# md-k-sarker/azure-hc-intel-tf

Measured on AMD Instinct MI355X. Metric: images/sec (whole node) ResNet-50 bs=64/worker at 1/2/4/8 MI355X, higher is better.
Workload: dtype fp32; 1 GPU; model=resnet50, global_batch=64, per_gpu_batch=64, image_size=224, parallelism=dp1, optimizer=momentum(0.9)+wd4e-5, fp32 master, graph=True, backward_segments=stage, kernels=hip

## Files before the change

### azure_hc_intel_tf_amd/ops/autotune.py

```python
from __future__ import annotations

import json
import math
import os
from typing import Dict, List, Tuple

import torch

from . import _ext
from . import functional as Fn

_DIR = os.path.join(os.path.dirname(os.path.dirname(os.path.abspath(__file__))), "tuned")


def _table_path(v):
    if not v or os.path.isabs(v) or os.path.exists(v):
        return v
    alt = os.path.join(os.path.dirname(os.path.dirname(os.path.dirname(os.path.abspath(__file__)))), v)
    return alt if os.path.exists(alt) else v


DEFAULT_CACHE = _table_path(os.environ.get("HCB_TUNED_TABLE")) or os.path.join(_DIR, "mi355x.json")
CACHE_VERSION = 6


def _entry_valid(key, val) -> bool:
    tiles = {"fwd": Fn._CONV_TILES, "dgb": Fn._CONV_TILES, "wgrad": Fn._WGRAD_TILES, "fwd3": Fn._P3_TILES,
             "wgrad3": Fn._WP3_TILES}.get(key[0])
    cfg, splits = (val[0], val[1]) if isinstance(val, (tuple, list)) else (val, 1)
    return tiles is not None and int(cfg) in tiles and int(splits) >= 1


def _key_str(k) -> str:
    return "|".join(str(v) for v in k)


def _key_parse(s: str):
    parts = s.split("|")
    return (parts[0],) + tuple(int(p) for p in parts[1:])


def load_cache(path: str = DEFAULT_CACHE) -> int:
    if not os.path.exists(path):
        return 0
    with open(path) as f:
        d = json.load(f)
    if d.get("version") != CACHE_VERSION:
        return 0
    table = {}
    for k, v in d.get("entries", {}).items():
        key, val = _key_parse(k), tuple(v) if isinstance(v, list) else v
        if _entry_valid(key, val):
# ... 117 lines not shown


def layer_problems_p3(layer, batch: int, dev) -> List[Tuple]:
    spec = layer.spec
    H, W, Cin = layer.in_shape
    P, Q, Cout = layer.out_shape
    N = batch
    M = N * P * Q
    taps = spec.kh * spec.kw
    geo = Fn.dgrad_problem(spec, N, H, W, P, Q)
    phases = Fn.dgrad_phases(spec, H, W) if layer.need_dx and Fn.uses_dgrad_phases(spec, H, W) else []
    buf = {}

    def ops():
        if not buf:
            buf["x"] = _planes((N, H, W, Cin), dev)
            buf["dz"] = _planes((N, P, Q, Cout), dev)
            buf["y"] = torch.empty((N, P, Q, Cout), dtype=torch.float32, device=dev)
            buf["acc"] = torch.zeros(8 * 2 * Cout, dtype=torch.float32, device=dev)
            buf["dx"] = torch.zeros((N, H, W, Cin), dtype=torch.float32, device=dev)
            buf["dw"] = torch.zeros((Cout, spec.K), dtype=torch.float32, device=dev)
        return buf

    out = [(Fn.fwd3_key(M, Cout, spec.K, taps), [list(c) for c in Fn.p3_candidates(M, Cout, spec.K)],
            lambda plan: Fn.conv_forward(ops()["x"], spec, layer.pack.pack, None, ops()["y"], stats=ops()["acc"],
                                         cfg=plan, stats_R=8))]
    if layer.need_dx:
        if not phases:
            out.append((Fn.fwd3_key(geo[0], Cin, geo[1], taps), [list(c) for c in Fn.p3_candidates(geo[0], Cin, geo[1])],
                        lambda plan: Fn.conv_dgrad(ops()["dz"], spec, layer.pack.tr, None, ops()["dx"], False,
                                                   cfg=plan)))
        for ph in phases:
            pm, pk, pt = Fn.dgrad_phase_problem(spec, N, ph)
            out.append((Fn.fwd3_key(pm, Cin, pk, pt), [list(c) for c in Fn.p3_candidates(pm, Cin, pk)],
                        lambda plan, ph=ph: Fn.dgrad_phase(ops()["dz"], spec, layer.pack.tr, ops()["dx"], True, ph,
                                                           cfg=plan)))
    out.append((Fn.wgrad3_key(Cout, spec.K, M, taps), [list(c) for c in Fn.wgrad_p3_candidates(Cout, spec.K, M)],
                lambda plan: Fn.conv_wgrad(ops()["dz"], ops()["x"], spec, ops()["dw"], cfg=tuple(plan))))
    return out


def _best(cands, run):
    best = None
    for plan in cands:
        t = _time(lambda: run(plan))
        if best is None or t < best[0]:
            best = (t, plan)
    return best


def model_problems(model, batch: int):
    from ..nn.layers import ConvBN
# ... 63 lines not shown
```

### azure_hc_intel_tf_amd/ops/functional.py

```python
from __future__ import annotations

import math
import os
from dataclasses import dataclass
from typing import NamedTuple

import torch
import torch.nn.functional as F

from . import _ext


def ld(t) -> int:
    if t.dim() == 4:
        assert t.stride(3) == 1, "activation channels must be contiguous"
        return t.stride(2)
    assert t.dim() == 2 and t.stride(1) == 1
    return t.stride(0)


def _round_up(x: int, m: int) -> int:
    return (x + m - 1) // m * m


# ... 428 lines not shown


def dgrad_problem(spec, N, H, W, P, Q):
    return dgrad_geom(spec, N, H, W, P, Q, 0, 0)[1][:2]


def set_tuned(table: dict) -> None:
    _tuned.update(table)


_P3_TILES = {0: (128, 64), 1: (64, 128), 2: (128, 64), 3: (64, 128), 4: (64, 64), 5: (128, 64), 6: (64, 128),
             7: (128, 128), 8: (128, 128), 9: (128, 128), 10: (256, 128), 11: (128, 256), 12: (64, 128),
             13: (128, 64), 14: (128, 64), 15: (64, 128), 16: (64, 64), 17: (64, 64),
             18: (64, 128), 19: (128, 64), 20: (64, 64), 21: (64, 64), 22: (128, 128),
             23: (64, 128), 24: (128, 64), 25: (64, 64), 26: (64, 64), 27: (128, 128), 28: (128, 128),
             31: (64, 256), 32: (128, 256), 33: (64, 64), 34: (128, 64),
             35: (128, 64), 36: (128, 128)}
_P3_OCC = {14: 2, 15: 2, 16: 2, 17: 3, 18: 2, 19: 2, 20: 2, 21: 3, 23: 2, 24: 2, 25: 2, 26: 3}
_P3_PERSIST = {18: 15, 19: 14, 20: 16, 21: 17, 22: 7, 23: 15, 24: 14, 25: 16, 26: 17, 27: 7, 28: 8,
               31: 15, 32: 15, 33: 16, 34: 14, 35: 14, 36: 7}
_P3_BRES = {31: 3, 32: 2, 33: 3, 34: 2, 35: 2, 36: 2}


def p3_bres_fits(cfg: int, N: int, K: int) -> bool:
    bm, bn = _P3_TILES[cfg]
    kpad = -(-K // 64) * 64
    return _P3_BRES[cfg] * 3 * bm * 64 + kpad * 3 * bn * 2 + 4 * N <= 160 * 1024
_P3_STREAMK = {23: 18, 24: 19, 25: 20, 26: 21, 27: 22, 28: 8}
_WP3_TILES = {0: (128, 64), 1: (64, 128), 2: (64, 64), 3: (128, 64), 4: (64, 128), 5: (64, 64),
              6: (128, 128), 7: (128, 128), 8: (256, 128), 9: (128, 256), 10: (128, 128), 11: (128, 64),
              12: (128, 64), 13: (64, 128), 14: (64, 64), 15: (64, 64),
              16: (128, 64), 17: (64, 128), 18: (64, 64)}
_WP3_OCC = {12: 2, 13: 2, 14: 2, 15: 3, 16: 2, 17: 2, 18: 3}


def fwd3_key(M: int, N: int, K: int, taps: int = 1):
    return ("fwd3", M, N, K, taps)


def wgrad3_key(Nout: int, K: int, M: int, taps: int = 1):
    return ("wgrad3", Nout, K, M, taps)


def p3_candidates(M: int, N: int, K: int):
    out = []
    ksteps = math.ceil(K / 64)
# ... 310 lines not shown

    def __init__(self, mean, invstd):
        self.mean = mean
        self.invstd = invstd


def conv_bn_inference(x, spec: ConvSpec, wpack, w_master, gamma, beta, running_mean, running_var, eps, out,
                      relu: bool, residual=None, cfg=None):
    N, H, W, _ = x.shape
    P, Q = spec.out_hw(H, W)
    M = N * P * Q
    p3 = is_planes(x) or (native(x) and x.dtype == torch.float32)
    if not p3 and not native(x):
        z = torch.empty((N, P, Q, spec.cout), dtype=out.dtype, device=x.device)
        conv_forward(x, spec, wpack, w_master, z)
        return bn_inference(z, gamma, beta, running_mean, running_var, eps, out, relu, residual=residual)
    if p3:
        x = to_planes(x)
        assert out.dtype == torch.float32, "fp32 conv needs an fp32 (or Planes) output"
        if residual is not None:
            residual = to_planes(residual) if is_planes(out) else from_planes(residual)
    cfg, splits = _plan(cfg, M, spec.cout, spec.K, x.device, spec.kh * spec.kw, **(_P3_PLAN if p3 else {}))
    if p3:
        cfg = _P3_PERSIST.get(cfg, cfg)
    elif cfg in PATCH_CFGS:
        cfg, splits = _PATCH_TWIN[cfg], 1
    if residual is not None:
        assert ld(residual) == ld(out) and residual.shape == out.shape and residual.dtype == out.dtype
    geom = fwd_geom(spec, N, H, W, ld(x), ld(out), residual is not None, not is_planes(out) and _f32o(out), relu)
    _launch(x, wpack, out, geom, cfg, splits, yres=residual, inf=(gamma, beta, running_mean, running_var, float(eps)))
    return out


def bn_inference(z, gamma, beta, running_mean, running_var, eps, out, relu: bool, residual=None):
    N, H, W, C = z.shape
    if native(z) and z.dtype == torch.float32:
        M = N * H * W
        acc = torch.stack([torch.zeros_like(running_var), running_var * float(M)]).unsqueeze(0).contiguous()
        scratch = torch.empty(2, C, dtype=torch.float32, device=z.device)
        if residual is not None:
            if is_planes(out) and not is_planes(residual):
                residual = to_planes(residual)
            elif not is_planes(out) and is_planes(residual):
                residual = from_planes(residual)
        _ext.ops().bn_apply_acc(z, ld(z), _pl(out), ld(out), _pl(residual), ld(residual) if residual is not None else 0,
                                M, C, acc, 1, eps, 1.0, gamma, beta, 1 if relu else 0, scratch[0], scratch[1],
                                None, None, running_mean)
# ... 390 lines not shown
```

### csrc/bindings.cpp

```cpp
#include <algorithm>
#include <vector>

#include <torch/library.h>
#include <ATen/core/Tensor.h>
#include <ATen/ops/empty.h>
#include <c10/hip/HIPStream.h>
#include <c10/util/Exception.h>

#include "kernels/kernels.h"

using at::Tensor;

#ifdef HCB_F16
constexpr at::ScalarType kAct = at::kHalf;
#define HCB_ACT_NAME "float16"
#else
constexpr at::ScalarType kAct = at::kBFloat16;
#define HCB_ACT_NAME "bfloat16"
#endif
#define HCB_TORCH_LIBRARY(ns, m) TORCH_LIBRARY(ns, m)
#define HCB_TORCH_LIBRARY_IMPL(ns, k, m) TORCH_LIBRARY_IMPL(ns, k, m)

namespace {

// ... 276 lines not shown
    TORCH_CHECK(t->dim() == 1 && t->numel() == p.Nout && t->is_contiguous() && t->device() == y.device(),
                "hcb.conv_inf: gamma / beta / moving mean / moving variance must be fp32 [cout] on the output's device");
  }
  p.bnb_gamma = gamma.data_ptr<float>();
  p.bnb_beta = beta.data_ptr<float>();
  p.bnb_mean = mean.data_ptr<float>();
  p.bnb_invstd = var.data_ptr<float>();
  p.inf = 1;
  p.inf_eps = (float)eps;
}

void conv_igemm_inf(const Tensor& x, const Tensor& w, const Tensor& y, const c10::optional<Tensor>& res,
                    at::IntArrayRef g, int64_t cfg, const Tensor& gamma, const Tensor& beta, const Tensor& mean,
                    const Tensor& var, double eps) {
  TORCH_CHECK(hcb::conv_cfg_has_inf((int)cfg), "hcb.conv_igemm_inf: cfg 0..16 (a patch cfg runs its LDS-DMA twin)");
  hcb::ConvParams p = igemm_params(x, w, y, res, c10::nullopt, c10::nullopt, g, cfg);
  TORCH_CHECK(x.scalar_type() != at::kFloat && !p.out_f32,
              "hcb.conv_igemm_inf: 16-bit operands and output (fp32 runs on the plane GEMMs: hcb.conv_p3_inf)");
  TORCH_CHECK(!p.beta || res->scalar_type() == y.scalar_type(), "hcb.conv_igemm_inf: res dtype differs from y");
  set_inf(p, y, gamma, beta, mean, var, eps);
  hcb::launch_conv_igemm(p, (int)cfg, cur_stream());
}

std::vector<int64_t> gemm_cfg_table(std::string family) {
  const hcb::GemmCfg* rows = nullptr;
  int n = 0;
  bool (*inf)(int) = [](int) { return false; };
  if (family == "conv") {
    rows = hcb::CONV_CFGS, n = hcb::N_CONV_CFG, inf = hcb::conv_cfg_has_inf;
  } else if (family == "wgrad") {
    rows = hcb::WGRAD_CFGS, n = hcb::N_WGRAD_CFG;
  } else if (family == "p3") {
    rows = hcb::P3_CFGS, n = hcb::N_P3_CFG, inf = hcb::p3_cfg_has_inf;
  } else if (family == "wgrad_p3") {
    rows = hcb::WP3_CFGS, n = hcb::N_WP3_CFG;
  } else {
    TORCH_CHECK(false, "hcb.gemm_cfg_table: family is conv, wgrad, p3 or wgrad_p3");
  }
  std::vector<int64_t> out;
  for (int i = 0; i < n; ++i) {
    const hcb::GemmCfg& r = rows[i];
    for (int v : {r.cfg, r.kind, r.wm, r.wn, r.tm, r.tn, r.kw, r.nst, r.occ, r.extra, r.fb, (int)inf(i)}) out.push_back(v);
  }
  return out;
}

int wgrad_params(hcb::WgradParams& p, const Tensor& dy, const Tensor& x, const Tensor& dw, at::IntArrayRef g,
                 int64_t splits, const char* op) {
  p = decode_geom(kWgradGeom, g, op);
  check_f32(dw, "dw");
  p.K = p.R * p.S * p.C;
  TORCH_CHECK(p.C % 8 == 0 && p.ldx % 8 == 0, "hcb.", op, ": C, ldx multiples of 8");
  TORCH_CHECK(p.ldy % 8 == 0 && p.ldy >= p.Nout, "hcb.", op, ": bad ldy");
  TORCH_CHECK(splits >= 1, "hcb.", op, ": splits >= 1");
  const int64_t xb = x_span_bytes(p.N, p.H, p.W, p.C, p.ldx, 2);
  const int64_t yb = out_span_bytes(p.M, p.ldy, p.Nout, 2);
  TORCH_CHECK(xb < (1ll << 31) && yb < (1ll << 31), "hcb.", op, ": operand exceeds 2 GiB");
  check_range(dw, (int64_t)p.Nout * p.K * 4, "dw");
  const int nkt = (p.M + 63) / 64;
  const int per = (nkt + (int)splits - 1) / (int)splits;
// ... 686 lines not shown
  const bool p3 = wp.dim() == 3 && wp.size(0) == 3 && wp.scalar_type() == at::kBFloat16;
  TORCH_CHECK((p3 || wp.scalar_type() == kAct) && wp.is_contiguous() && wp.numel() == (p3 ? 3 : 1) * w.size(0) * 256,
              "hcb.stem_wfold: wp bf16 [cout][256] or planes [3][cout][256]");
  hcb::launch_stem_wfold(w.data_ptr<float>(), (int)w.size(0), (int)w.size(3),
                         reinterpret_cast<uint16_t*>(wp.data_ptr()), cur_stream(), p3);
}

void stem_wgrad_unfold(const Tensor& dwp, const Tensor& dw) {
  check_f32(dwp, "dwp");
  check_f32(dw, "dw");
  TORCH_CHECK(dw.dim() == 4 && dw.size(1) == 7 && dw.size(2) == 7 && dw.size(3) >= 3 && dw.is_contiguous() &&
                  dwp.is_contiguous() && dwp.numel() == dw.size(0) * 256,
              "hcb.stem_wgrad_unfold: dwp [cout][256] -> dw [cout][7][7][>=3]");
  hcb::launch_stem_wgrad_unfold(dwp.data_ptr<float>(), (int)dw.size(0), (int)dw.size(3), dw.data_ptr<float>(),
                                cur_stream());
}


hcb::ConvParams p3_params(const Tensor& x, const Tensor& w, const Tensor& w_lo, const Tensor& y,
                          const c10::optional<Tensor>& yres, const c10::optional<Tensor>& bias,
                          const c10::optional<Tensor>& stats, at::IntArrayRef g, int64_t cfg,
                          const c10::optional<Tensor>& stats_shift, bool y_planes = false) {
  const int64_t xps = check_planes(x, "x");
  TORCH_CHECK(cfg >= 0 && cfg < hcb::N_P3_CFG, "hcb.conv_p3: cfg 0..36");
  hcb::ConvParams p = conv_params(x.select(0, 0), w, y, yres, bias, g);
  const int bm = hcb::p3_tile_m((int)cfg), bn = hcb::p3_tile_n((int)cfg);
  TORCH_CHECK(y_planes ? !p.out_f32 : p.out_f32 && y.scalar_type() == at::kFloat,
              "hcb.conv_p3: fp32 output (geom out_f32 = 0 with a plane output)");
  check_range(x, 2 * xps * 2 + (int64_t)p.x_bytes, "x planes");
  TORCH_CHECK(2 * xps * 2 < (1ll << 32), "hcb.conv_p3: plane stride exceeds the 32-bit offset range");
  p.x_plane = (uint32_t)(xps * 2);
  TORCH_CHECK(w_lo.dim() == 2 && w_lo.size(0) == 2 && w_lo.stride(1) == 1 && w_lo.scalar_type() == w.scalar_type() &&
                  w_lo.size(1) >= (int64_t)p.Nout * p.Kpad,
              "hcb.conv_p3: w_lo must be [2][>= Nout*Kpad] of the pack's type");
  const Tensor m = w_lo.select(0, 0), l = w_lo.select(0, 1);
  check_align16(m.data_ptr(), "w_lo[0]");
  check_align16(l.data_ptr(), "w_lo[1]");
  p.w_lo = m.data_ptr();
  p.w_lo2 = l.data_ptr();
  attach_stats(p, stats, bm, "conv_p3");
  TORCH_CHECK(!stats_shift.has_value() || p.stats != nullptr, "hcb.conv_p3: stats_shift without stats");
  p.stats_shift = opt_f32(stats_shift, p.Nout, "stats_shift");
  attach_splitk(p, bm, bn, "conv_p3");
  if (hcb::p3_cfg_streamk((int)cfg)) {
    TORCH_CHECK(g_splitk_ws != nullptr && g_splitk_cnt != nullptr, "hcb.conv_p3: stream-K needs the split-K workspace");
    p.ws = g_splitk_ws;
    p.cnt = g_splitk_cnt;
// ... 90 lines not shown
  hcb::launch_merge_planes((const uint16_t*)in.data_ptr(), (int)ldi, ps, rows, (int)C, y.data_ptr<float>(), (int)ldy,
                           cur_stream());
}

void gap_fwd_p3(const Tensor& x, const Tensor& y, int64_t N, int64_t HW, int64_t C) {
  const int64_t xps = check_planes(x, "x"), yps = check_planes(y, "y");
  TORCH_CHECK(C % 8 == 0, "hcb.gap_fwd_p3: C % 8");
  check_range(x, (2 * xps + N * HW * C) * 2, "x");
  check_range(y, (2 * yps + N * C) * 2, "y");
  hcb::launch_gap_fwd_p3((const uint16_t*)x.data_ptr(), xps, (uint16_t*)y.data_ptr(), yps, (int)N, (int)HW, (int)C,
                         cur_stream());
}

void set_deterministic(bool on) { hcb::set_deterministic(on); }

}


HCB_TORCH_LIBRARY(hcb, m) {
  m.def("conv_igemm(Tensor x, Tensor w, Tensor(a!) y, Tensor? yres, Tensor? bias, Tensor(b!)? stats, int[] geom, int cfg, Tensor? stats_shift=None) -> ()");
  m.def("conv_igemm_bnb(Tensor x, Tensor w, Tensor(a!) y, Tensor? yres, int[] geom, int cfg, Tensor z, Tensor? yact, int ld, Tensor mean, Tensor invstd, Tensor gamma, Tensor beta, Tensor(b!) acc, int R, int mode) -> ()");
  m.def("conv_igemm_inf(Tensor x, Tensor w, Tensor(a!) y, Tensor? res, int[] geom, int cfg, Tensor gamma, Tensor beta, Tensor mean, Tensor var, float eps) -> ()");
  m.def("gemm_cfg_table(str family) -> int[]", gemm_cfg_table);
  m.def("conv_geom_fields(str kind) -> str[]", conv_geom_fields);
  m.def("set_splitk_workspace(Tensor ws, Tensor cnt) -> ()");
  m.def("set_p3p_bnb(int v) -> ()", set_p3p_bnb);
  m.def("conv_wgrad(Tensor dy, Tensor x, Tensor(a!) dw, int[] geom, int cfg, int splits) -> ()");
  m.def("bn_apply(Tensor x, int ldx, Tensor(a!) y, int ldy, Tensor? res, int ldr, int M, int C, Tensor mean, Tensor invstd, Tensor gamma, Tensor beta, int relu) -> ()");
  m.def("pool_fwd(Tensor x, Tensor(a!) y, Tensor(b!)? idx, int[] geom) -> ()");
  m.def("pool_bwd(Tensor dy, Tensor x, Tensor y, Tensor? idx, Tensor(a!) dx, int[] geom, bool accumulate) -> ()");
  m.def("pool_fwd_p3(Tensor x, Tensor(a!) y, Tensor(b!)? idx, int[] geom) -> ()");
  m.def("gap_fwd(Tensor x, Tensor(a!) y, int N, int HW, int C) -> ()");
  m.def("gap_bwd(Tensor dy, Tensor(a!) dx, int N, int HW, int C) -> ()");
  m.def("softmax_xent(Tensor logits, int ld, Tensor labels, int ncls, Tensor(a!) row_loss, Tensor(b!) dlogits, int lddl, float scale, Tensor? scale_dev=None, Tensor(c!)? dl32=None, float label_smoothing=0.0) -> ()");
  m.def("eval_metrics(Tensor logits, int ld, Tensor labels, int ncls, Tensor(a!) counters) -> ()");
  m.def("nonfinite(Tensor g, Tensor(a!) flag) -> ()");
  m.def("loss_total(Tensor row_loss, int B, Tensor? l2, float half_wd, Tensor(a!) loss) -> ()");
  m.def("loss_scale_update(Tensor(a!) hyper, float world, bool dynamic) -> ()");
  m.def("colsum(Tensor g, int ld, int M, int N, Tensor(a!) out) -> ()");
  m.def("zero_bufs(Tensor(a!)[] ts) -> ()");
  m.def("sgd_momentum(Tensor(a!) w, Tensor(b!) mom, Tensor g, int n_decay, Tensor hyper, Tensor(c!)? l2, bool nesterov) -> ()");
  m.def("rmsprop(Tensor(a!) w, Tensor(b!) mom, Tensor(c!) ms, Tensor g, int n_decay, Tensor hyper, Tensor ohyper, Tensor(d!)? l2) -> ()");
  m.def("adam(Tensor(a!) w, Tensor(b!) m, Tensor(c!) v, Tensor g, int n_decay, Tensor hyper, Tensor ohyper, Tensor state, Tensor(d!)? l2) -> ()");
  m.def("adam_advance(Tensor(a!) state, Tensor ohyper, Tensor hyper) -> ()");
  m.def("weight_pack(Tensor master, Tensor(a!) pack, Tensor table, int max_work, int lo=0) -> ()");
  m.def("add_bf16(Tensor a, Tensor b, Tensor(a!) y) -> ()");
// ... 78 lines not shown
```

### csrc/kernels/conv_p3.hip

```cpp
#include "conv_p3_fwd.h"
#include "conv_p3_persist.h"
#include "conv_p3_wgrad.h"

namespace hcb {

#define HCB_CASE_TILE(...)
#define HCB_CASE_PERSIST(C, WM, WN, TM, TN, KW, NST, OCC, FB) \
  case C: return launch_p3p<WM, WN, TM, TN, KW, NST, OCC>(p, st) ? -1 : launch_p3_persist(p, FB, st);
#define HCB_CASE_STREAMK(C, WM, WN, TM, TN, KW, NST, OCC, FB) \
  case C: return launch_p3sk<WM, WN, TM, TN, KW, NST, OCC>(p, st) ? -1 : launch_p3_persist(p, FB, st);
#define HCB_CASE_BRES(C, WM, WN, TM, TN, KW, NST, OCC, FB) \
  case C: return launch_p3bres<WM, WN, TM, TN, KW, NST>(p, st) ? -1 : launch_p3_persist(p, FB, st);
#define HCB_CASE_RETIRED(C, WM, WN, TM, TN, KW, NST, OCC, FB) \
  case C: return launch_p3_persist(p, FB, st);
static int launch_p3_persist(const ConvParams& p, int cfg, hipStream_t st) {
  switch (cfg) {
    HCB_P3_CFGS(HCB_CASE)
    default: return cfg;
  }
}
#undef HCB_CASE_TILE
#undef HCB_CASE_PERSIST
#undef HCB_CASE_STREAMK
#undef HCB_CASE_BRES
#undef HCB_CASE_RETIRED

void set_p3p_bnb(int v) { p3p_bnb_level() = v; }

void launch_conv_p3(const ConvParams& p, int cfg, hipStream_t st) {
  if (p.inf) {
    launch_p3_cfg<false, true>(p, cfg, st);
    return;
  }
  if (cfg >= 0 && (cfg = launch_p3_persist(p, cfg, st)) < 0) return;
  if (p.bnb_acc != nullptr)
    launch_p3_cfg<true, false>(p, cfg, st);
  else
    launch_p3_cfg<false, false>(p, cfg, st);
}

#define HCB_CASE_TILE(C, WM, WN, TM, TN, KW, NST, OCC) \
  case C: wlaunch_p3<WM, WN, TM, TN, NST, KW, OCC>(p, splits, st); break;
#define HCB_CASE_PERSIST(C, WM, WN, TM, TN, KW, NST, OCC) \
  case C: wlaunch_p3p<WM, WN, TM, TN, OCC>(p, splits, st); break;
void launch_wgrad_p3(const WgradParams& p, int cfg, int splits, hipStream_t st) {
  switch (cfg) {
    HCB_WP3_CFGS(HCB_CASE)
    default: launch_wgrad_p3(p, 2, splits, st); break;
  }
}
#undef HCB_CASE_TILE
#undef HCB_CASE_PERSIST

__global__ __launch_bounds__(256) void split_planes_kernel(const float* __restrict__ x, int ldx, int C, int64_t n8,
                                                           uint16_t* __restrict__ out, int ldo, int64_t plane) {
  const int CV = C >> 3;
// ... 75 lines not shown
```

### csrc/kernels/gemm_cfg.h

```cpp
#pragma once

namespace hcb {

enum GemmKind {
  K_REG = 0,
  K_GLDS = 1,
  K_PATCH = 2,
  K_KQ = 3,
  K_TILE = 4,
  K_PERSIST = 5,
  K_STREAMK = 6,
  K_BRES = 7,
  K_RETIRED = 8,
};

#define HCB_CONV_CFGS(X)                  \
  X(0, REG, 2, 2, 64, 64, 0, 0, -1)       \
  X(1, REG, 4, 1, 32, 64, 0, 0, -1)       \
  X(2, REG, 2, 2, 32, 32, 0, 0, -1)       \
  X(3, REG, 1, 4, 64, 32, 0, 0, -1)       \
  X(4, GLDS, 2, 2, 64, 64, 3, 0, -1)      \
  X(5, GLDS, 4, 1, 32, 64, 3, 0, -1)      \
  X(6, GLDS, 2, 2, 32, 32, 4, 0, -1)      \
  X(7, GLDS, 1, 4, 64, 32, 3, 0, -1)      \
  X(8, GLDS, 2, 2, 64, 64, 4, 0, -1)      \
  X(9, GLDS, 2, 2, 64, 64, 5, 0, -1)      \
  X(10, GLDS, 4, 1, 32, 64, 6, 0, -1)     \
  X(11, GLDS, 1, 4, 64, 32, 6, 0, -1)     \
  X(12, GLDS, 2, 4, 64, 32, 3, 0, -1)     \
  X(13, GLDS, 4, 2, 32, 64, 3, 0, -1)     \
  X(14, GLDS, 4, 2, 64, 64, 3, 0, -1)     \
  X(15, GLDS, 2, 4, 64, 64, 3, 0, -1)     \
  X(16, GLDS, 2, 4, 32, 32, 4, 0, -1)     \
  X(17, PATCH, 2, 4, 64, 32, 3, 8, 13)    \
  X(18, PATCH, 4, 2, 64, 64, 3, 8, 14)    \
  X(19, PATCH, 4, 2, 64, 32, 3, 8, 14)    \
// ... 36 lines not shown
  X(15, TILE, 2, 2, 32, 64, 32, 2, 2, -1)       \
  X(16, TILE, 2, 2, 32, 32, 32, 3, 2, -1)       \
  X(17, TILE, 2, 2, 32, 32, 32, 2, 3, -1)       \
  X(18, PERSIST, 2, 2, 32, 64, 32, 2, 2, 15)    \
  X(19, PERSIST, 2, 2, 64, 32, 32, 2, 2, 14)    \
  X(20, PERSIST, 2, 2, 32, 32, 32, 3, 2, 16)    \
  X(21, PERSIST, 2, 2, 32, 32, 32, 2, 3, 17)    \
  X(22, PERSIST, 2, 4, 64, 32, 32, 3, 1, 7)     \
  X(23, STREAMK, 2, 2, 32, 64, 32, 2, 2, 18)    \
  X(24, STREAMK, 2, 2, 64, 32, 32, 2, 2, 19)    \
  X(25, STREAMK, 2, 2, 32, 32, 32, 3, 2, 20)    \
  X(26, STREAMK, 2, 2, 32, 32, 32, 2, 3, 21)    \
  X(27, STREAMK, 2, 4, 64, 32, 32, 3, 1, 22)    \
  X(28, STREAMK, 4, 2, 32, 64, 32, 3, 1, 8)     \
  X(29, RETIRED, 4, 2, 64, 64, 32, 2, 1, 10)    \
  X(30, RETIRED, 2, 4, 64, 64, 32, 2, 1, 11)    \
  X(31, BRES, 1, 4, 64, 64, 32, 3, 1, 18)       \
  X(32, BRES, 2, 4, 64, 64, 32, 2, 1, 18)       \
  X(33, BRES, 2, 2, 32, 32, 32, 3, 1, 20)       \
  X(34, BRES, 2, 2, 64, 32, 32, 2, 1, 19)       \
  X(35, BRES, 4, 2, 32, 32, 32, 2, 1, 19)       \
  X(36, BRES, 4, 2, 32, 64, 32, 2, 1, 22)

#define HCB_WP3_CFGS(X)                   \
  X(0, TILE, 2, 2, 64, 32, 64, 2, 1)      \
  X(1, TILE, 2, 2, 32, 64, 64, 2, 1)      \
  X(2, TILE, 2, 2, 32, 32, 64, 3, 1)      \
  X(3, TILE, 4, 2, 32, 32, 64, 2, 1)      \
  X(4, TILE, 2, 4, 32, 32, 64, 2, 1)      \
  X(5, TILE, 2, 2, 32, 32, 64, 2, 1)      \
  X(6, TILE, 2, 4, 64, 32, 32, 3, 1)      \
  X(7, TILE, 4, 2, 32, 64, 32, 3, 1)      \
  X(8, TILE, 4, 2, 64, 64, 32, 2, 1)      \
  X(9, TILE, 2, 4, 64, 64, 32, 2, 1)      \
  X(10, TILE, 2, 2, 64, 64, 32, 3, 1)     \
  X(11, TILE, 2, 2, 64, 32, 32, 3, 1)     \
  X(12, TILE, 2, 2, 64, 32, 32, 2, 2)     \
  X(13, TILE, 2, 2, 32, 64, 32, 2, 2)     \
  X(14, TILE, 2, 2, 32, 32, 32, 3, 2)     \
  X(15, TILE, 2, 2, 32, 32, 32, 2, 3)     \
  X(16, PERSIST, 2, 2, 64, 32, 32, 2, 2)  \
  X(17, PERSIST, 2, 2, 32, 64, 32, 2, 2)  \
  X(18, PERSIST, 2, 2, 32, 32, 32, 2, 3)

#define HCB_CASE(C, KIND, ...) HCB_CASE_##KIND(C, __VA_ARGS__)

struct GemmCfg {
  int cfg, kind, wm, wn, tm, tn, kw, nst, occ, extra, fb;
};

#define HCB_ROW_CONV(C, KIND, WM, WN, TM, TN, NST, PMAX, FB) {C, K_##KIND, WM, WN, TM, TN, 64, NST, 1, PMAX, FB},
#define HCB_ROW_WGRAD(C, KIND, WM, WN, TM, TN, NST, KS) {C, K_##KIND, WM, WN, TM, TN, 64, NST, 1, KS, -1},
#define HCB_ROW_P3(C, KIND, WM, WN, TM, TN, KW, NST, OCC, FB) {C, K_##KIND, WM, WN, TM, TN, KW, NST, OCC, 0, FB},
#define HCB_ROW_WP3(C, KIND, WM, WN, TM, TN, KW, NST, OCC) {C, K_##KIND, WM, WN, TM, TN, KW, NST, OCC, 0, -1},
inline constexpr GemmCfg CONV_CFGS[] = {HCB_CONV_CFGS(HCB_ROW_CONV)};
inline constexpr GemmCfg WGRAD_CFGS[] = {HCB_WGRAD_CFGS(HCB_ROW_WGRAD)};
inline constexpr GemmCfg P3_CFGS[] = {HCB_P3_CFGS(HCB_ROW_P3)};
inline constexpr GemmCfg WP3_CFGS[] = {HCB_WP3_CFGS(HCB_ROW_WP3)};
#undef HCB_ROW_CONV
#undef HCB_ROW_WGRAD
#undef HCB_ROW_P3
#undef HCB_ROW_WP3

template <int N>
constexpr bool gemm_cfgs_in_order(const GemmCfg (&t)[N]) {
  for (int i = 0; i < N; ++i)
    if (t[i].cfg != i || t[i].fb >= N) return false;
  return true;
}
static_assert(gemm_cfgs_in_order(CONV_CFGS) && gemm_cfgs_in_order(WGRAD_CFGS) && gemm_cfgs_in_order(P3_CFGS) &&
                  gemm_cfgs_in_order(WP3_CFGS),
              "row i of a table is cfg i, and falls back inside the table");

constexpr int N_CONV_CFG = sizeof(CONV_CFGS) / sizeof(GemmCfg);
constexpr int N_WGRAD_CFG = sizeof(WGRAD_CFGS) / sizeof(GemmCfg);
constexpr int N_P3_CFG = sizeof(P3_CFGS) / sizeof(GemmCfg);
constexpr int N_WP3_CFG = sizeof(WP3_CFGS) / sizeof(GemmCfg);

template <int N>
constexpr int gemm_kind(const GemmCfg (&t)[N], int cfg) {
  return cfg >= 0 && cfg < N ? t[cfg].kind : -1;
}
template <int N>
constexpr int gemm_tile(const GemmCfg (&t)[N], int cfg, bool n, int d) {
  return cfg < 0 || cfg >= N ? d : n ? t[cfg].wn * t[cfg].tn : t[cfg].wm * t[cfg].tm;
}
constexpr int conv_tile_m(int cfg) { return gemm_tile(CONV_CFGS, cfg, false, 128); }
constexpr int conv_tile_n(int cfg) { return gemm_tile(CONV_CFGS, cfg, true, 128); }
constexpr int wgrad_tile_m(int cfg) { return gemm_tile(WGRAD_CFGS, cfg, false, 64); }
constexpr int wgrad_tile_n(int cfg) { return gemm_tile(WGRAD_CFGS, cfg, true, 64); }
constexpr int p3_tile_m(int cfg) { return gemm_tile(P3_CFGS, cfg, false, 128); }
constexpr int p3_tile_n(int cfg) { return gemm_tile(P3_CFGS, cfg, true, 64); }
constexpr int p3_slot_k(int cfg) { return cfg >= 0 && cfg < N_P3_CFG ? P3_CFGS[cfg].kw : 32; }
constexpr int wgrad_p3_tile_m(int cfg) { return gemm_tile(WP3_CFGS, cfg, false, 64); }
constexpr int wgrad_p3_tile_n(int cfg) { return gemm_tile(WP3_CFGS, cfg, true, 64); }

constexpr bool conv_cfg_has_inf(int cfg) { return cfg >= 0 && cfg < N_CONV_CFG && CONV_CFGS[cfg].kind != K_PATCH; }
constexpr bool p3_cfg_has_inf(int cfg) { return gemm_kind(P3_CFGS, cfg) == K_TILE; }
constexpr bool conv_cfg_splitk(int cfg) { return cfg >= 0 && gemm_kind(CONV_CFGS, cfg) != K_REG; }
constexpr bool p3_cfg_streamk(int cfg) {
  return gemm_kind(P3_CFGS, cfg) == K_STREAMK || gemm_kind(P3_CFGS, cfg) == K_RETIRED;
}
constexpr bool wp3_cfg_persistent(int cfg) { return gemm_kind(WP3_CFGS, cfg) == K_PERSIST; }

}
```

Measured before the change: 4266 images/sec.

## Add patch-staged 3x3 implicit-GEMM conv kernel reusing input halo across taps

New measurement: 4316 images/sec (median of 6 runs). 1.01x the previous value.

```diff
diff --git a/azure_hc_intel_tf_amd/ops/autotune.py b/azure_hc_intel_tf_amd/ops/autotune.py
--- a/azure_hc_intel_tf_amd/ops/autotune.py
+++ b/azure_hc_intel_tf_amd/ops/autotune.py
@@ -28,6 +28,8 @@
     tiles = {"fwd": Fn._CONV_TILES, "dgb": Fn._CONV_TILES, "wgrad": Fn._WGRAD_TILES, "fwd3": Fn._P3_TILES,
              "wgrad3": Fn._WP3_TILES}.get(key[0])
     cfg, splits = (val[0], val[1]) if isinstance(val, (tuple, list)) else (val, 1)
+    if key[0] == "fwd3" and int(cfg) in Fn._P3_PATCH_TILES:
+        return key[4] == 9 and int(splits) == 1
     return tiles is not None and int(cfg) in tiles and int(splits) >= 1
 
 
@@ -191,12 +193,16 @@
             buf["dw"] = torch.zeros((Cout, spec.K), dtype=torch.float32, device=dev)
         return buf
 
-    out = [(Fn.fwd3_key(M, Cout, spec.K, taps), [list(c) for c in Fn.p3_candidates(M, Cout, spec.K)],
+    same = spec.sh == 1 and spec.sw == 1 and (P, Q) == (H, W)
+    patch = (lambda m, n, k: Fn.p3_patch_candidates(m, n, k, taps, H, W)) if same else (lambda m, n, k: [])
+    out = [(Fn.fwd3_key(M, Cout, spec.K, taps),
+            [list(c) for c in Fn.p3_candidates(M, Cout, spec.K) + patch(M, Cout, spec.K)],
             lambda plan: Fn.conv_forward(ops()["x"], spec, layer.pack.pack, None, ops()["y"], stats=ops()["acc"],
                                          cfg=plan, stats_R=8))]
     if layer.need_dx:
         if not phases:
-            out.append((Fn.fwd3_key(geo[0], Cin, geo[1], taps), [list(c) for c in Fn.p3_candidates(geo[0], Cin, geo[1])],
+            out.append((Fn.fwd3_key(geo[0], Cin, geo[1], taps),
+                        [list(c) for c in Fn.p3_candidates(geo[0], Cin, geo[1]) + patch(geo[0], Cin, geo[1])],
                         lambda plan: Fn.conv_dgrad(ops()["dz"], spec, layer.pack.tr, None, ops()["dx"], False,
                                                    cfg=plan)))
         for ph in phases:
diff --git a/azure_hc_intel_tf_amd/ops/functional.py b/azure_hc_intel_tf_amd/ops/functional.py
--- a/azure_hc_intel_tf_amd/ops/functional.py
+++ b/azure_hc_intel_tf_amd/ops/functional.py
@@ -474,6 +474,30 @@
 _P3_BRES = {31: 3, 32: 2, 33: 3, 34: 2, 35: 2, 36: 2}
 
 
+_P3_PATCH_TILES = {64: (128, 128)}
+_P3_PATCH_FB = {64: 8}
+_P3_PATCH_NST = 3
+
+
+def p3_patch_rows(H: int, W: int, bm: int) -> int:
+    d = bm - 1
+    span = d + (d + W - 1) // W + (W + 1) * ((d + H * W - 1) // (H * W)) + 2 * (W + 1) + 3
+    return -(-span // 16) * 16
+
+
+def p3_patch_fits(cfg: int, H: int, W: int, bnb: bool = True) -> bool:
+    bm, bn = _P3_PATCH_TILES[cfg]
+    lds = _P3_PATCH_NST * 3 * bn * 64 + 2 * 3 * p3_patch_rows(H, W, bm) * 64 + 1024 + (bn * 16 if bnb else 0)
+    return lds <= 160 * 1024
+
+
+def p3_patch_candidates(M: int, N: int, K: int, taps: int, H: int, W: int):
+    if taps != 9 or K % (9 * 32) != 0:
+        return []
+    return [(c, 1) for c, (bm, bn) in _P3_PATCH_TILES.items()
+            if not (N <= 64 and bn > 64) and p3_patch_fits(c, H, W)]
+
+
 def p3_bres_fits(cfg: int, N: int, K: int) -> bool:
     bm, bn = _P3_TILES[cfg]
     kpad = -(-K // 64) * 64
@@ -830,7 +854,7 @@
             residual = to_planes(residual) if is_planes(out) else from_planes(residual)
     cfg, splits = _plan(cfg, M, spec.cout, spec.K, x.device, spec.kh * spec.kw, **(_P3_PLAN if p3 else {}))
     if p3:
-        cfg = _P3_PERSIST.get(cfg, cfg)
+        cfg = _P3_PERSIST.get(_P3_PATCH_FB.get(cfg, cfg), _P3_PATCH_FB.get(cfg, cfg))
     elif cfg in PATCH_CFGS:
         cfg, splits = _PATCH_TWIN[cfg], 1
     if residual is not None:
diff --git a/csrc/bindings.cpp b/csrc/bindings.cpp
--- a/csrc/bindings.cpp
+++ b/csrc/bindings.cpp
@@ -322,6 +322,13 @@
   hcb::launch_conv_igemm(p, (int)cfg, cur_stream());
 }
 
+std::vector<int64_t> p3_patch_fit(int64_t cfg, int64_t H, int64_t W, bool bnb) {
+  TORCH_CHECK(hcb::p3_cfg_patch((int)cfg) && H >= 1 && W >= 1 && H < 32768 && W < 32768, "hcb.p3_patch_fit: a patch cfg, H, W >= 1");
+  const int bm = hcb::p3_tile_m((int)cfg);
+  return {(int64_t)hcb::p3_patch_cfg_lds((int)cfg, (int)H, (int)W, bnb), (int64_t)hcb::p3_patch_rows((int)H, (int)W, bm),
+          (int64_t)hcb::P3_PATCH_LDS_MAX};
+}
+
 std::vector<int64_t> gemm_cfg_table(std::string family) {
   const hcb::GemmCfg* rows = nullptr;
   int n = 0;
@@ -334,8 +341,10 @@
     rows = hcb::P3_CFGS, n = hcb::N_P3_CFG, inf = hcb::p3_cfg_has_inf;
   } else if (family == "wgrad_p3") {
     rows = hcb::WP3_CFGS, n = hcb::N_WP3_CFG;
+  } else if (family == "p3_patch") {
+    rows = hcb::P3PATCH_CFGS, n = hcb::N_P3PATCH_CFG;
   } else {
-    TORCH_CHECK(false, "hcb.gemm_cfg_table: family is conv, wgrad, p3 or wgrad_p3");
+    TORCH_CHECK(false, "hcb.gemm_cfg_table: family is conv, wgrad, p3, wgrad_p3 or p3_patch");
   }
   std::vector<int64_t> out;
   for (int i = 0; i < n; ++i) {
@@ -1068,7 +1077,7 @@
                           const c10::optional<Tensor>& stats, at::IntArrayRef g, int64_t cfg,
                           const c10::optional<Tensor>& stats_shift, bool y_planes = false) {
   const int64_t xps = check_planes(x, "x");
-  TORCH_CHECK(cfg >= 0 && cfg < hcb::N_P3_CFG, "hcb.conv_p3: cfg 0..36");
+  TORCH_CHECK(hcb::p3_cfg_valid((int)cfg), "hcb.conv_p3: cfg 0..36, or a 3x3 patch cfg (64..)");
   hcb::ConvParams p = conv_params(x.select(0, 0), w, y, yres, bias, g);
   const int bm = hcb::p3_tile_m((int)cfg), bn = hcb::p3_tile_n((int)cfg);
   TORCH_CHECK(y_planes ? !p.out_f32 : p.out_f32 && y.scalar_type() == at::kFloat,
@@ -1205,6 +1214,7 @@
   m.def("conv_igemm_bnb(Tensor x, Tensor w, Tensor(a!) y, Tensor? yres, int[] geom, int cfg, Tensor z, Tensor? yact, int ld, Tensor mean, Tensor invstd, Tensor gamma, Tensor beta, Tensor(b!) acc, int R, int mode) -> ()");
   m.def("conv_igemm_inf(Tensor x, Tensor w, Tensor(a!) y, Tensor? res, int[] geom, int cfg, Tensor gamma, Tensor beta, Tensor mean, Tensor var, float eps) -> ()");
   m.def("gemm_cfg_table(str family) -> int[]", gemm_cfg_table);
+  m.def("p3_patch_fit(int cfg, int H, int W, bool bnb) -> int[]", p3_patch_fit);
   m.def("conv_geom_fields(str kind) -> str[]", conv_geom_fields);
   m.def("set_splitk_workspace(Tensor ws, Tensor cnt) -> ()");
   m.def("set_p3p_bnb(int v) -> ()", set_p3p_bnb);
diff --git a/csrc/kernels/conv_p3.hip b/csrc/kernels/conv_p3.hip
--- a/csrc/kernels/conv_p3.hip
+++ b/csrc/kernels/conv_p3.hip
@@ -1,4 +1,5 @@
 #include "conv_p3_fwd.h"
+#include "conv_p3_patch.h"
 #include "conv_p3_persist.h"
 #include "conv_p3_wgrad.h"
 
@@ -32,6 +33,7 @@
     launch_p3_cfg<false, true>(p, cfg, st);
     return;
   }
+  if (p3_cfg_patch(cfg) && (cfg = launch_p3_patch_cfg(p, cfg, st)) < 0) return;
   if (cfg >= 0 && (cfg = launch_p3_persist(p, cfg, st)) < 0) return;
   if (p.bnb_acc != nullptr)
     launch_p3_cfg<true, false>(p, cfg, st);
diff --git a/csrc/kernels/conv_p3_patch.h b/csrc/kernels/conv_p3_patch.h
--- /dev/null
+++ b/csrc/kernels/conv_p3_patch.h
@@ -0,0 +1,247 @@
+#pragma once
+#include "conv_p3_fwd.h"
+#include "gemm_cfg.h"
+
+namespace hcb {
+
+__device__ __forceinline__ int p3p_lp(const ConvParams& p, int m) {
+  const int n = (int)fdiv((uint32_t)m, p.fd_hw), r = m - n * p.H * p.W;
+  const int pp = (int)fdiv((uint32_t)r, p.fd_w), qq = r - pp * p.W;
+  return (n * (p.H + 1) + pp) * (p.W + 1) + qq;
+}
+
+template <int BN, int NST>
+constexpr int p3p_ring_bytes() {
+  return NST * NPL * BN * 64;
+}
+template <int BN, int NST, int NT>
+constexpr int p3p_pmax() {
+  const int rows = (int)((P3_PATCH_LDS_MAX - p3p_ring_bytes<BN, NST>() - 1024 - BN * 16) / (2 * NPL * 64));
+  return (rows + NT / 4 - 1) / (NT / 4);
+}
+
+template <int WM, int WN, int TM, int TN, int NST, bool BNB>
+__global__ __launch_bounds__(WM* WN * 64, WM* WN / 4) void conv_p3_patch_kernel(ConvParams p) {
+  constexpr int BM = WM * TM, BN = WN * TN;
+  constexpr int MI = TM / 16, NI = TN / 16;
+  constexpr int NT = WM * WN * 64, RB = 64, RP = NT / 4;
+  constexpr int BV = BN / RP;
+  constexpr int LW = NPL * BV;
+  constexpr int PMAX = p3p_pmax<BN, NST, NT>();
+  constexpr int PL = NPL * PMAX;
+  constexpr int BIMG = BN * RB, BSTAGE = NPL * BIMG;
+  static_assert(BV >= 1 && BV * RP == BN, "weight tile rows must be a multiple of the load pass");
+  static_assert(NST >= 3 && NST <= 4 && (NST - 1) * LW + PL <= 63, "vmcnt range");
+  static_assert(igemm_epilogue_lds(BM, BN, WM) <= (size_t)p3p_ring_bytes<BN, NST>() + 2 * NPL * 16 * RB,
+                "the epilogue staging must lie below the BN parameters");
+  extern __shared__ __attribute__((aligned(16))) char smem[];
+
+  const int tid = threadIdx.x, lane = tid & 63;
+  const int wid = wave_id_uniform();
+  const int wm = wid / WN, wn = wid % WN;
+  const int tiles_n = (p.Nout + BN - 1) / BN;
+  const int tile = xcd_remap(blockIdx.x, gridDim.x);
+  const int tm = tile / tiles_n, tn = tile % tiles_n;
+  const int m0 = tm * BM, n0 = tn * BN;
+  const int chunk = (tid & 3) ^ p3_swz<32>(tid >> 2);
+  const int W1 = p.W + 1;
+
+  const int prows_max = p.patch_rows;
+  const int pimg = prows_max * RB;
+  char* ring = smem;
+  char* patch = smem + NST * BSTAGE;
+  char* sink = patch + 2 * NPL * pimg;
+  const size_t param_off = (size_t)(NST * BSTAGE + 2 * NPL * pimg + 1024);
+
+  const char* xb = reinterpret_cast<const char*>(p.x);
+  const __amdgpu_buffer_rsrc_t xr0 = make_rsrc(xb, p.x_bytes);
+  const __amdgpu_buffer_rsrc_t xr1 = make_rsrc(xb + p.x_plane, p.x_bytes);
+  const __amdgpu_buffer_rsrc_t xr2 = make_rsrc(xb + 2 * (size_t)p.x_plane, p.x_bytes);
+  const __amdgpu_buffer_rsrc_t wr0 = make_rsrc(p.w, p.w_bytes);
+  const __amdgpu_buffer_rsrc_t wr1 = make_rsrc(p.w_lo, p.w_bytes);
+  const __amdgpu_buffer_rsrc_t wr2 = make_rsrc(p.w_lo2, p.w_bytes);
+
+  const int mlast = min(m0 + BM, p.M) - 1;
+  const int lbase = p3p_lp(p, m0);
+  const int reach = 2 * W1 + 3;
+  const int prows = min(p3p_lp(p, mlast) + reach - lbase, prows_max);
+  uint32_t poff[PMAX];
+  {
+    const int HW1 = (p.H + 1) * W1;
+#pragma unroll
+    for (int v = 0; v < PMAX; ++v) {
+      const int j = v * RP + (tid >> 2);
+      uint32_t o = HCB_OOB;
+      if (j < prows) {
+        const int L = lbase + j;
+        const int n = (int)fdiv((uint32_t)L, p.fd_hw2), rem = L - n * HW1;
+        const int hh = (int)fdiv((uint32_t)rem, p.fd_w2), ww = rem - hh * W1;
+        if (n < p.N && hh >= 1 && ww >= 1)
+          o = (uint32_t)((((n * p.H + hh - 1) * p.W + ww - 1) * p.ldx + chunk * 8) * 2);
+      }
+      poff[v] = o;
+    }
+  }
+  int prow[MI];
+#pragma unroll
+  for (int i = 0; i < MI; ++i) {
+    const int m = m0 + wm * TM + i * 16 + (lane & 15);
+    prow[i] = min(p3p_lp(p, m <= mlast ? m : mlast) - lbase, prows_max - reach);
+  }
+  uint32_t b_off[BV];
+#pragma unroll
+  for (int v = 0; v < BV; ++v) {
+    const int j = n0 + (tid >> 2) + RP * v;
+    b_off[v] = (j < p.Nout) ? (uint32_t)(j * p.Kpad + chunk * 8) * 2u : HCB_OOB;
+  }
+
+  const int nslab = p.C / 32, nk = nslab * 9;
+
+  f32x4 acc[MI][NI];
+#pragma unroll
+  for (int i = 0; i < MI; ++i)
+#pragma unroll
+    for (int j = 0; j < NI; ++j) acc[i][j] = f32x4{0.f, 0.f, 0.f, 0.f};
+
+  EpiPrefetch<WM, WN, TM, TN, BNB, true> pre;
+  pre.load_shift(p, n0, wn, lane);
+  if constexpr (BNB) stage_bnb_params<BN, NT>(p, n0, smem + param_off);
+
+  auto load_patch = [&](int sl) {
+    char* pb = patch + (sl & 1) * NPL * pimg;
+    const uint32_t cb = (uint32_t)sl * 64u;
+#pragma unroll
+    for (int v = 0; v < PMAX; ++v) {
+      const int row0 = v * RP + wid * 16;
+      const bool in = row0 < prows_max;
+      const uint32_t o = (in && poff[v] != HCB_OOB) ? poff[v] + cb : HCB_OOB;
+      char* d = pb + row0 * RB;
+      glds16(xr0, in ? d : sink, o);
+      glds16(xr1, in ? d + pimg : sink, o);
+      glds16(xr2, in ? d + 2 * pimg : sink, o);
+    }
+  };
+  auto issue_w = [&](int stage, int sl, int t) {
+    const bool live = sl < nslab;
+    const uint32_t kb = (uint32_t)(t * p.C + sl * 32) * 2u;
+    char* sb = ring + stage * BSTAGE + wid * 16 * RB;
+#pragma unroll
+    for (int v = 0; v < BV; ++v) {
+      const uint32_t o = (b_off[v] == HCB_OOB || !live) ? HCB_OOB : b_off[v] + kb;
+      glds16(wr0, sb + RP * v * RB, o);
+      glds16(wr1, sb + BIMG + RP * v * RB, o);
+      glds16(wr2, sb + 2 * BIMG + RP * v * RB, o);
+    }
+  };
+  const int frow = lane & 15, fq = lane >> 4;
+  auto read = [&](int stage, int sl, int t, P3Frags<TM, TN, 1>& f) {
+    const int r = t / 3, tapoff = r * W1 + (t - 3 * r);
+    const u32x4* A = reinterpret_cast<const u32x4*>(patch + (sl & 1) * NPL * pimg);
+    const u32x4* B = reinterpret_cast<const u32x4*>(ring + stage * BSTAGE);
+    const int aimg = prows_max * 4;
+#pragma unroll
+    for (int i = 0; i < MI; ++i) {
+      const int row = prow[i] + tapoff, o = row * 4 + (fq ^ p3_swz<32>(row));
+#pragma unroll
+      for (int t3 = 0; t3 < NPL; ++t3) f.a[0][t3][i] = A[t3 * aimg + o];
+    }
+#pragma unroll
+    for (int j = 0; j < NI; ++j) {
+      const int row = wn * TN + j * 16 + frow, o = row * 4 + (fq ^ p3_swz<32>(row));
+#pragma unroll
+      for (int t3 = 0; t3 < NPL; ++t3) f.b[0][t3][j] = B[t3 * (BIMG / 16) + o];
+    }
+  };
+
+  load_patch(0);
+#pragma unroll
+  for (int s = 0; s < NST; ++s) issue_w(s, s / 9, s % 9);
+  P3Frags<TM, TN, 1> fr[2];
+  wait_vmcnt<(NST - 1) * LW>();
+  __builtin_amdgcn_s_barrier();
+  asm volatile("" ::: "memory");
+  read(0, 0, 0, fr[0]);
+
+  constexpr int NMF = MI * NI * 6, NRD = (MI + NI) * NPL;
+  int sl = 0, t = 0, st = 0;
+  int slr = NST / 9, tr = NST % 9;
+  auto body = [&](P3Frags<TM, TN, 1>& cur, P3Frags<TM, TN, 1>& nxt) {
+    const bool has_next = sl + 1 < nslab;
+    asm volatile("s_waitcnt lgkmcnt(0)" ::: "memory");
+    if (has_next && t >= 1 && t <= NST - 2)
+      wait_vmcnt<(NST - 2) * LW + PL>();
+    else
+      wait_vmcnt<(NST - 2) * LW>();
+    __builtin_amdgcn_s_barrier();
+    asm volatile("" ::: "memory");
+    if (has_next && t == 0) load_patch(sl + 1);
+    issue_w(st, slr, tr);
+    int sn = sl, tn1 = t + 1, stn = st + 1;
+    if (tn1 == 9) {
+      tn1 = 0;
+      ++sn;
+    }
+    if (stn == NST) stn = 0;
+    read(stn, sn, tn1, nxt);
+    p3_mma<TM, TN, 1>(cur, acc);
+    ilv_schedule<NMF, LW, NRD>();
+    sl = sn;
+    t = tn1;
+    st = stn;
+    if (++tr == 9) {
+      tr = 0;
+      ++slr;
+    }
+  };
+  for (int k = 0; k < nk; k += 2) {
+    body(fr[0], fr[1]);
+    if (k + 1 < nk) body(fr[1], fr[0]);
+  }
+  asm volatile("s_waitcnt vmcnt(0)" ::: "memory");
+  __syncthreads();
+  igemm_epilogue<WM, WN, TM, TN, BNB, true, false>(p, acc, smem, tm, m0, n0, wm, wn, lane, tid, pre, false,
+                                                   BNB ? smem + param_off : nullptr);
+}
+
+inline bool p3_patch_eligible(const ConvParams& p) {
+  return p.R == 3 && p.S == 3 && p.stride_h == 1 && p.stride_w == 1 && p.pad_h == 1 && p.pad_w == 1 &&
+         p.dil_h == 1 && p.dil_w == 1 && p.idil_h == 1 && p.idil_w == 1 && p.P == p.H && p.Q == p.W &&
+         p.C % 32 == 0 && p.Kpad >= 9 * p.C && !p.remap && p.splits == 1 && !p.inf && !p.y_p3 &&
+         p.w_lo != nullptr && p.w_lo2 != nullptr;
+}
+
+template <int WM, int WN, int TM, int TN, int NST>
+static bool launch_p3_patch(ConvParams p, hipStream_t st) {
+  constexpr int BM = WM * TM, BN = WN * TN, NT = WM * WN * 64;
+  if (!p3_patch_eligible(p)) return false;
+  const bool bnb = p.bnb_acc != nullptr;
+  const int rows = p3_patch_rows(p.H, p.W, BM);
+  const long lds = p3_patch_lds(p.H, p.W, BM, BN, NST, bnb);
+  if (lds > P3_PATCH_LDS_MAX || rows > p3p_pmax<BN, NST, NT>() * (NT / 4)) return false;
+  p.patch_rows = rows;
+  p.fd_hw = make_fastdiv((uint32_t)(p.H * p.W));
+  p.fd_w = make_fastdiv((uint32_t)p.W);
+  p.fd_hw2 = make_fastdiv((uint32_t)((p.H + 1) * (p.W + 1)));
+  p.fd_w2 = make_fastdiv((uint32_t)(p.W + 1));
+  static const hipError_t once[2] = {set_lds_max(conv_p3_patch_kernel<WM, WN, TM, TN, NST, false>),
+                                     set_lds_max(conv_p3_patch_kernel<WM, WN, TM, TN, NST, true>)};
+  (void)once;
+  const int tiles = ((p.M + BM - 1) / BM) * ((p.Nout + BN - 1) / BN);
+  if (bnb)
+    hipLaunchKernelGGL((conv_p3_patch_kernel<WM, WN, TM, TN, NST, true>), dim3(tiles), dim3(NT), (size_t)lds, st, p);
+  else
+    hipLaunchKernelGGL((conv_p3_patch_kernel<WM, WN, TM, TN, NST, false>), dim3(tiles), dim3(NT), (size_t)lds, st, p);
+  return true;
+}
+
+#define HCB_CASE_P3PATCH(C, WM, WN, TM, TN, KW, NST, OCC, FB) \
+  case C: return launch_p3_patch<WM, WN, TM, TN, NST>(p, st) ? -1 : FB;
+static int launch_p3_patch_cfg(const ConvParams& p, int cfg, hipStream_t st) {
+  switch (cfg) {
+    HCB_P3PATCH_CFGS(HCB_CASE)
+    default: return cfg;
+  }
+}
+#undef HCB_CASE_P3PATCH
+
+}
diff --git a/csrc/kernels/gemm_cfg.h b/csrc/kernels/gemm_cfg.h
--- a/csrc/kernels/gemm_cfg.h
+++ b/csrc/kernels/gemm_cfg.h
@@ -12,6 +12,7 @@
   K_STREAMK = 6,
   K_BRES = 7,
   K_RETIRED = 8,
+  K_P3PATCH = 9,
 };
 
 #define HCB_CONV_CFGS(X)                  \
@@ -94,6 +95,9 @@
   X(35, BRES, 4, 2, 32, 32, 32, 2, 1, 19)       \
   X(36, BRES, 4, 2, 32, 64, 32, 2, 1, 22)
 
+constexpr int P3_PATCH_CFG0 = 64;
+#define HCB_P3PATCH_CFGS(X) X(64, P3PATCH, 4, 2, 32, 64, 32, 3, 1, 8)
+
 #define HCB_WP3_CFGS(X)                   \
   X(0, TILE, 2, 2, 64, 32, 64, 2, 1)      \
   X(1, TILE, 2, 2, 32, 64, 64, 2, 1)      \
@@ -129,6 +133,7 @@
 inline constexpr GemmCfg WGRAD_CFGS[] = {HCB_WGRAD_CFGS(HCB_ROW_WGRAD)};
 inline constexpr GemmCfg P3_CFGS[] = {HCB_P3_CFGS(HCB_ROW_P3)};
 inline constexpr GemmCfg WP3_CFGS[] = {HCB_WP3_CFGS(HCB_ROW_WP3)};
+inline constexpr GemmCfg P3PATCH_CFGS[] = {HCB_P3PATCH_CFGS(HCB_ROW_P3)};
 #undef HCB_ROW_CONV
 #undef HCB_ROW_WGRAD
 #undef HCB_ROW_P3
@@ -148,6 +153,20 @@
 constexpr int N_WGRAD_CFG = sizeof(WGRAD_CFGS) / sizeof(GemmCfg);
 constexpr int N_P3_CFG = sizeof(P3_CFGS) / sizeof(GemmCfg);
 constexpr int N_WP3_CFG = sizeof(WP3_CFGS) / sizeof(GemmCfg);
+constexpr int N_P3PATCH_CFG = sizeof(P3PATCH_CFGS) / sizeof(GemmCfg);
+
+constexpr bool p3_patch_rows_ok() {
+  for (int i = 0; i < N_P3PATCH_CFG; ++i) {
+    const GemmCfg& r = P3PATCH_CFGS[i];
+    if (r.cfg != P3_PATCH_CFG0 + i || r.fb < 0 || r.fb >= N_P3_CFG || r.kw != 32) return false;
+    const GemmCfg& f = P3_CFGS[r.fb];
+    if (f.kind != K_TILE || f.wm * f.tm != r.wm * r.tm || f.wn * f.tn != r.wn * r.tn) return false;
+  }
+  return true;
+}
+static_assert(p3_patch_rows_ok(), "a patch row falls back to the per-tile cfg of the same block tile");
+constexpr bool p3_cfg_patch(int cfg) { return cfg >= P3_PATCH_CFG0 && cfg < P3_PATCH_CFG0 + N_P3PATCH_CFG; }
+constexpr bool p3_cfg_valid(int cfg) { return (cfg >= 0 && cfg < N_P3_CFG) || p3_cfg_patch(cfg); }
 
 template <int N>
 constexpr int gemm_kind(const GemmCfg (&t)[N], int cfg) {
@@ -161,8 +180,12 @@
 constexpr int conv_tile_n(int cfg) { return gemm_tile(CONV_CFGS, cfg, true, 128); }
 constexpr int wgrad_tile_m(int cfg) { return gemm_tile(WGRAD_CFGS, cfg, false, 64); }
 constexpr int wgrad_tile_n(int cfg) { return gemm_tile(WGRAD_CFGS, cfg, true, 64); }
-constexpr int p3_tile_m(int cfg) { return gemm_tile(P3_CFGS, cfg, false, 128); }
-constexpr int p3_tile_n(int cfg) { return gemm_tile(P3_CFGS, cfg, true, 64); }
+constexpr int p3_tile_m(int cfg) {
+  return p3_cfg_patch(cfg) ? gemm_tile(P3PATCH_CFGS, cfg - P3_PATCH_CFG0, false, 128) : gemm_tile(P3_CFGS, cfg, false, 128);
+}
+constexpr int p3_tile_n(int cfg) {
+  return p3_cfg_patch(cfg) ? gemm_tile(P3PATCH_CFGS, cfg - P3_PATCH_CFG0, true, 64) : gemm_tile(P3_CFGS, cfg, true, 64);
+}
 constexpr int p3_slot_k(int cfg) { return cfg >= 0 && cfg < N_P3_CFG ? P3_CFGS[cfg].kw : 32; }
 constexpr int wgrad_p3_tile_m(int cfg) { return gemm_tile(WP3_CFGS, cfg, false, 64); }
 constexpr int wgrad_p3_tile_n(int cfg) { return gemm_tile(WP3_CFGS, cfg, true, 64); }
@@ -175,4 +198,18 @@
 }
 constexpr bool wp3_cfg_persistent(int cfg) { return gemm_kind(WP3_CFGS, cfg) == K_PERSIST; }
 
-}
+constexpr int p3_patch_rows(int H, int W, int BM) {
+  const int d = BM - 1, span = d + (d + W - 1) / W + (W + 1) * ((d + H * W - 1) / (H * W)) + 2 * (W + 1) + 3;
+  return (span + 15) / 16 * 16;
+}
+constexpr long p3_patch_lds(int H, int W, int BM, int BN, int NST, bool bnb) {
+  return (long)NST * 3 * BN * 64 + 2l * 3 * p3_patch_rows(H, W, BM) * 64 + 1024 + (bnb ? BN * 16 : 0);
+}
+constexpr long p3_patch_cfg_lds(int cfg, int H, int W, bool bnb) {
+  if (!p3_cfg_patch(cfg)) return 0;
+  const GemmCfg& r = P3PATCH_CFGS[cfg - P3_PATCH_CFG0];
+  return p3_patch_lds(H, W, r.wm * r.tm, r.wn * r.tn, r.nst, bnb);
+}
+constexpr long P3_PATCH_LDS_MAX = 160 * 1024;
+
+}
```
